# xmarre/person_capture

Hardware: AMD Instinct MI355X
Metric: frames/sec detect+embed+match @1080p, 1/2/4/8 GPU; MFMA util % (higher is better)
Workload: dtype f16x3

## Files before the change

### include/pcgpu.h

```cpp
#ifndef PCGPU_H
#define PCGPU_H

#include <stddef.h>
#include <stdint.h>

#ifdef __cplusplus
extern "C" {
#endif

#define PC_ABI_VERSION 1

#define PC_OK 0
#define PC_ERR_ARG 1
#define PC_ERR_HIP 2
#define PC_ERR_STATE 3
#define PC_ERR_FORMAT 4
#define PC_ERR_CAPACITY 5

#define PC_PREC_F16 0
#define PC_PREC_F32 1
#define PC_PREC_F16X3 2

typedef struct pc_ctx pc_ctx;
typedef struct pc_net pc_net;
// ... 79 lines not shown
int pc_host_free(pc_ctx* ctx, void* h_ptr);
int pc_fence_create(pc_ctx* ctx, void** fence_out);
int pc_fence_record(pc_ctx* ctx, void* fence);
int pc_fence_wait(pc_ctx* ctx, void* fence);
int pc_fence_destroy(pc_ctx* ctx, void* fence);

int pc_net_create(pc_ctx* ctx, const void* h_program, size_t program_bytes, int precision, int max_batch,
                  pc_net** out);
int pc_net_destroy(pc_net* net);
int pc_net_run(pc_net* net, const void* d_input, int batch);
int pc_net_input_dims(pc_net* net, int32_t* h_dims4 );
int pc_net_output(pc_net* net, int index, void** d_ptr, int32_t* h_dims5 );
int pc_net_num_outputs(pc_net* net);
int pc_net_stats(pc_net* net, double* h_flops_per_image, int32_t* h_launches);
int pc_net_chain_info(pc_net* net, int32_t* h_min_batch, int32_t* h_images_per_round);
int pc_net_set_chain_min_batch(pc_net* net, int32_t min_batch);
int pc_net_set_graph(pc_net* net, int enable);
int pc_net_set_graph_max_batch(pc_net* net, int32_t max_batch);
int pc_net_profile(pc_net* net, int enable);
int pc_net_calibrate(pc_net* net, const void* d_in, int N, int headroom_log2, float* h_absmax);
int pc_net_profile_read(pc_net* net, double* h_out5);
int pc_net_profile_ops(pc_net* net, double* h_out, int max_recs);

int pc_letterbox(pc_ctx* ctx, int precision, const pc_letterbox_desc* h_descs, int n, int D, void* d_out);
int pc_warp_affine(pc_ctx* ctx, const pc_warp_desc* h_descs, int n);
int pc_resize_linear(pc_ctx* ctx, const pc_resize_desc* h_descs, int n);
int pc_face_quality(pc_ctx* ctx, const uint8_t* d_chips, int n, int side, double* d_out);
int pc_arcface_prep(pc_ctx* ctx, int precision, const uint8_t* d_chips, int n, int side, int flip, void* d_out);
int pc_rotate_pad(pc_ctx* ctx, const uint8_t* d_src, int H, int W, int row_stride, int deg, int pad, uint8_t* d_dst);
int pc_resize_area_fast(pc_ctx* ctx, const uint8_t* d_src, int row_stride, int isx, int isy, uint8_t* d_dst, int OH,
// ... 41 lines not shown
```

### person_capture_amd/_lib.py

```python
from __future__ import annotations

import ctypes as C
import os
from pathlib import Path

LIB_PATH = Path(os.environ.get("PC_LIB_PATH") or Path(__file__).resolve().parent / "lib" / "libpcgpu.so")

PC_OK = 0
PC_PREC_F16 = 0
PC_PREC_F32 = 1
PC_PREC_F16X3 = 2
PC_PREC_F16C8 = 3


def net_precision(mode: int) -> int:
    return PC_PREC_F16 if mode in (PC_PREC_F16X3, PC_PREC_F16C8) else mode

_lib = None


class LetterboxDesc(C.Structure):
    _fields_ = [("d_src", C.c_void_p), ("H", C.c_int32), ("W", C.c_int32), ("row_stride", C.c_int32),
                ("new_w", C.c_int32), ("new_h", C.c_int32), ("scale_x", C.c_double), ("scale_y", C.c_double),
                ("simd_end", C.c_int32), ("pad_", C.c_int32)]
# ... 61 lines not shown
    "pc_fence_create": ([_P, C.POINTER(_P)], _I),
    "pc_fence_record": ([_P, _P], _I),
    "pc_fence_wait": ([_P, _P], _I),
    "pc_fence_destroy": ([_P, _P], _I),
    "pc_net_create": ([_P, _P, _SZ, _I, _I, C.POINTER(_P)], _I),
    "pc_net_destroy": ([_P], _I),
    "pc_net_run": ([_P, _P, _I], _I),
    "pc_net_input_dims": ([_P, C.POINTER(C.c_int32)], _I),
    "pc_net_output": ([_P, _I, C.POINTER(_P), C.POINTER(C.c_int32)], _I),
    "pc_net_num_outputs": ([_P], _I),
    "pc_net_stats": ([_P, C.POINTER(C.c_double), C.POINTER(C.c_int32)], _I),
    "pc_ctx_wait_fence": ([_P, _P], _I),
    "pc_frame_stage": ([_P, _P, _P, C.c_size_t, C.c_size_t, C.c_size_t, C.c_int], _I),
    "pc_net_chain_info": ([_P, C.POINTER(C.c_int32), C.POINTER(C.c_int32)], _I),
    "pc_net_set_chain_min_batch": ([_P, C.c_int32], _I),
    "pc_net_set_graph": ([_P, _I], _I),
    "pc_net_set_graph_max_batch": ([_P, C.c_int32], _I),
    "pc_net_profile": ([_P, _I], _I),
    "pc_net_calibrate": ([_P, _P, _I, _I, C.POINTER(C.c_float)], _I),
    "pc_net_profile_read": ([_P, C.POINTER(C.c_double)], _I),
    "pc_net_profile_ops": ([_P, C.POINTER(C.c_double), _I], _I),
    "pc_letterbox": ([_P, _I, C.POINTER(LetterboxDesc), _I, _I, _P], _I),
    "pc_warp_affine": ([_P, C.POINTER(WarpDesc), _I], _I),
    "pc_resize_linear": ([_P, C.POINTER(ResizeDesc), _I], _I),
    "pc_face_quality": ([_P, _P, _I, _I, _P], _I),
    "pc_arcface_prep": ([_P, _I, _P, _I, _I, _I, _P], _I),
    "pc_rotate_pad": ([_P, _P, _I, _I, _I, _I, _I, _P], _I),
    "pc_resize_area_fast": ([_P, _P, _I, _I, _I, _P, _I, _I], _I),
    "pc_resize_area": ([_P, _P, _I, C.POINTER(AreaTab), C.POINTER(C.c_int32), _I, C.POINTER(AreaTab),
                        C.POINTER(C.c_int32), _I, _P, _I, _I], _I),
# ... 54 lines not shown
```

### person_capture_amd/csrc/pc_api.cpp

```cpp
#include <hip/hip_runtime.h>
#include <string.h>
#include <stdio.h>
#include <stdlib.h>
#include <string>
#include <vector>
#include <map>
#include <algorithm>
#include <thread>
#include <mutex>
#include <memory>
#include <cmath>
#include <atomic>
#include <condition_variable>
#include <functional>
#include <system_error>
#include "../../include/pcgpu.h"
#include "pc_common.h"

namespace pc {
hipError_t conv_launch(int f32, int rowb, int cfg, const ConvParams& p, hipStream_t s);
hipError_t conv_halo_launch(int f32, int cfg, const ConvParams& p, hipStream_t s);
hipError_t conv_fast_launch(int f32, int rowb, int cfg, const ConvParams& p, hipStream_t s);
hipError_t conv_hx_launch(const ConvParams& p, hipStream_t s);
hipError_t conv_hxg_launch(const ConvParams& p, int small, hipStream_t s);
hipError_t conv_hxi_launch(const ConvParams& p, int small, hipStream_t s);
int conv_fast_num_cfgs();
constexpr int kFastSmallCfg0 = 15, kFastSmallCfg1 = 19;
int conv_fast_tile(int cfg, int* bc, int* bp);
int conv_fast_valid(int cfg, int rowb);
int conv_fast_valid_sx(int cfg, int rowb);
int conv_fast_valid_c8(int cfg, int rowb);
int conv_fast_valid_wg(int cfg);
int conv_halo_num_cfgs();
int conv_halo_tile(int cfg, int* bc, int* bp);
int conv_halo_fits(int cfg, int KH, int KW, int W);
hipError_t conv_t2d_launch(const ConvParams& p, int variant, hipStream_t s);
int conv_t2d_select(int cin, int npad, int KH, int KW, int stride, int pad, int act, int out_f32, int ycs,
                    int ycoff, int split);
int conv_t2d_rows(int variant);
int conv_chain_fits(int H, int W, int C, int npad, long long ktot);
// ... 481 lines not shown
  int split = 0;
  void* w = nullptr;
  float* bias = nullptr;
  float* slope = nullptr;
};
struct ProfRec { int a, b, kind; double flops; int op = -1; int code = -1; int small = -1; };
struct ChainBlockH { const void* w1; const float* b1; const float* s1; const void* w2; const float* b2; };
struct ChainPlan {
  int first = -1, nblk = 0, in_t = -1, out_t = -1;
  void* d_blk = nullptr;
  void* d_wpack = nullptr;
  int wl = 0;
  double flops_per_image = 0.0;
};

struct pc_net {
  pc_ctx* ctx = nullptr;
  int f32 = 0;
  int max_batch = 0;
  int in_tensor = 0;
  int in_centered = 0;
  std::vector<NetBuf> bufs;
  std::vector<NetTensor> tens;
  std::vector<NetOp> ops;
  std::vector<int> outs;
  std::vector<void*> arrays;
  std::vector<long long> array_count;
  std::vector<ConvPlan> plans;
  std::vector<std::vector<ConvPlan>> plans_cls;
  std::vector<int> cls_batch;
  std::vector<StemPlan> stems;
  std::vector<ChainPlan> chains;
  std::vector<int> chain_at;
  int chain_min_batch = 32;
  int attn_stream = 0;
  std::vector<const float*> host_arrays;
  void* stem_col = nullptr;
  float* partial = nullptr;
  size_t partial_bytes = 0;
  double flops_per_image = 0.0;
  int launches = 0;
  const void* cur_input = nullptr;
  void* in_copy = nullptr;
  size_t in_img_bytes = 0;
  int use_graph = 0;
  int capturing = 0;
  hipStream_t cap_stream = nullptr;
  std::mutex graph_mu;
  int graph_max_batch = 1 << 30;
// ... 19 lines not shown
    return (void*)(base + (size_t)T.coff * esize(n, T.is_f32));
  }
  return (char*)n->bufs[T.buf].d + (size_t)T.coff * esize(n, T.is_f32);
}

static const size_t kZeroTail = 65536;

static unsigned tensor_zero_off(const pc_net* n, int t) {
  const NetTensor& T = n->tens[t];
  const int es = esize(n, T.is_f32);
  const size_t end = T.buf < 0 ? n->in_img_bytes * n->max_batch : (size_t)n->bufs[T.buf].elems * n->max_batch * es;
  return (unsigned)(end - (size_t)T.coff * es);
}

static const int kNumConvCfgs = 14;

static int c8_rowb() {
  const char* e = getenv("PC_C8_ROWB");
  return e && atoi(e) == 128 ? 128 : 64;
}

static int plan_conv(pc_net* n, const NetOp& op, ConvPlan& pl, long long plan_batch, bool small = false) {
  const int* w = op.w;
  const int out = w[1], nseg = w[2], npad = w[14];
  const int esz = n->f32 ? 4 : 2;
  int rowb = 128;
  bool any_split = n->tens[out].split != 0 || (w[21] >= 0 && n->tens[w[21]].split);
  for (int s = 0; s < nseg; ++s) {
    const NetTensor& X = n->tens[w[3 + 5 * s]];
    const int cl = X.split ? X.C / 2 : X.C;
// ... 174 lines not shown
    }
    const bool c224 = X.C == 448 && Y.H == 20 && plan_batch <= 16;
    if (X.split && !X.c8 && !Y.c8 && (X.C == 192 || c224) && X.cs == X.C && Y.split && Y.C == X.C && npad == X.C / 2 &&
        w[4] == 3 && w[5] == 3 && w[6] == 1 && w[7] == 1 && X.H == Y.H && X.W == Y.W && w[15] == 27 * npad &&
        !(w[21] >= 0 && (w[22] == RES_UP2 || !n->tens[w[21]].split || n->tens[w[21]].c8)) &&
        (double)X.H * X.W * n->max_batch * X.cs * esz + kZeroTail < 4294967296.0 &&
        !(getenv("PC_CONV_HXG") && atoi(getenv("PC_CONV_HXG")) == 0)) {
      const int hxg_mask = getenv("PC_CONV_HXG") ? atoi(getenv("PC_CONV_HXG")) : 3;
      if (plan_batch * ((Y.H + 19) / 20) * ((Y.W + 15) / 16) >= 128 && (hxg_mask & 1) && !c224) pl.hx = 2;
      else if ((hxg_mask & 2) && (Y.H >= 40 || plan_batch <= 16)) pl.hx = 5;
    }
    if (pl.hx == 2 || pl.hx == 5) {
      pl.fast = pl.halo = pl.t2d = -1;
      pl.sx = 0;
    }
    const int hxi_mask = getenv("PC_CONV_HXI") ? atoi(getenv("PC_CONV_HXI")) : 59;
    if (!X.split && !X.c8 && !X.is_f32 && !Y.split && !Y.is_f32 && !Y.c8 && X.cs == X.C && Y.cs == Y.C && Y.C == X.C &&
        npad == X.C && w[4] == 3 && w[5] == 3 && w[6] == 1 && w[7] == 1 && X.W == X.H && Y.H == X.H && Y.W == X.W &&
        w[15] == 9 * X.C && !(w[21] >= 0 && (w[22] == RES_UP2 || n->tens[w[21]].split || n->tens[w[21]].is_f32)) &&
        (((hxi_mask & 4) && X.C == 256 && X.H == 14 && plan_batch >= 192) ||
         ((hxi_mask & 8) && X.C == 128 && X.H == 28 && plan_batch >= 64)) &&
        (double)X.H * X.W * n->max_batch * X.cs * esz + kZeroTail < 4294967296.0) {
      pl.hx = X.C == 256 ? 3 : 4;
      pl.fast = pl.halo = pl.t2d = -1;
      pl.sx = 0;
    }
    const int hc = X.C / 2;
    const bool hxs_shape = (hxi_mask & 32) && plan_batch <= 32 &&
                           ((hc == 256 && X.H == 14) || (hc == 128 && X.H == 28) || (hc == 512 && X.H == 7));
    const bool hxi_shape = ((hxi_mask & 1) && hc == 256 && X.H == 14 && plan_batch >= 192) ||
                           ((hxi_mask & 2) && hc == 128 && X.H == 28 && plan_batch >= 64) ||
// ... 187 lines not shown
    }
    for (int k = 0; k < ch.nblk; ++k) {
      const int* a = n->ops[i + 2 * k].w;
      const int* b = n->ops[i + 2 * k + 1].w;
      const void* w1 = ch.wl ? (const void*)((char*)ch.d_wpack + cbytes * (2 * k)) : n->arrays[a[13]];
      const void* w2 = ch.wl ? (const void*)((char*)ch.d_wpack + cbytes * (2 * k + 1)) : n->arrays[b[13]];
      hb[k] = ChainBlockH{w1, (const float*)n->arrays[a[17]], (const float*)n->arrays[a[19]], w2,
                          (const float*)n->arrays[b[17]]};
      ch.flops_per_image += n->plans[i + 2 * k].flops_per_image + n->plans[i + 2 * k + 1].flops_per_image;
    }
    HIPCHK(n->ctx, hipMalloc(&ch.d_blk, hb.size() * sizeof(ChainBlockH)));
    HIPCHK(n->ctx, hipMemcpy(ch.d_blk, hb.data(), hb.size() * sizeof(ChainBlockH), hipMemcpyHostToDevice));
    n->chain_at[i] = (int)n->chains.size();
    n->chains.push_back(ch);
    i += 2 * ch.nblk;
  }
  return PC_OK;
}

static uint8_t e4m3_encode(float v) {
  const uint8_t sgn = std::signbit(v) ? 0x80 : 0;
  const float a = std::fabs(v);
  if (!(a == a)) return 0x7f;
  if (a >= 448.f) return sgn | 0x7e;
  int e2 = 0;
  std::frexp(a, &e2);
  int E = e2 - 1;
  if (a == 0.f || E < -6) {
    const int q = (int)std::nearbyint(std::ldexp(a, 9));
    return sgn | (uint8_t)q;
// ... 306 lines not shown
      n->flops_per_image += 4.0 * T * T * op.w[3] * op.w[4];
      n->launches += 1;
    } else {
      rc = fail(c, PC_ERR_FORMAT, "unknown op type");
    }
  }
  n->wfrag.assign(n->ops.size(), nullptr);
  for (size_t i = 0; i < n->ops.size() && rc == PC_OK; ++i) {
    if (n->ops[i].w[0] != OP_CONV) continue;
    bool wg = n->plans[i].wg || n->plans[i].hx;
    for (auto& pc : n->plans_cls) wg = wg || pc[i].wg || pc[i].hx;
    if (wg) rc = pack_wfrag(n, n->ops[i], reinterpret_cast<const float*>(n->host_arrays[n->ops[i].w[13]]), &n->wfrag[i]);
  }
  n->host_arrays.clear();
  if (rc == PC_OK) rc = plan_chains(n);
  if (rc == PC_OK && stem_col_bytes) {
    if (hipMalloc(&n->stem_col, stem_col_bytes) != hipSuccess) rc = fail(c, PC_ERR_HIP, "stem im2col workspace");
    else hipMemset(n->stem_col, 0, stem_col_bytes);
  }
  if (rc == PC_OK && part) {
    if (hipMalloc((void**)&n->partial, part) != hipSuccess) rc = fail(c, PC_ERR_HIP, "split-K workspace");
    n->partial_bytes = part;
  }
  if (rc != PC_OK) {
    pc_net_destroy(n);
    return rc;
  }
  *out = n;
  return PC_OK;
}
// ... 5 lines not shown
  for (auto& kv : n->graphs) hipGraphExecDestroy(kv.second);
  if (n->cap_stream) hipStreamDestroy(n->cap_stream);
  if (n->d_absmax) hipFree(n->d_absmax);
  for (void* a : n->arrays) if (a) hipFree(a);
  for (void* a : n->wfrag) if (a) hipFree(a);
  for (auto& b : n->bufs) if (b.d) hipFree(b.d);
  if (n->partial) hipFree(n->partial);
  if (n->prep) hipFree(n->prep);
  if (n->in_copy) hipFree(n->in_copy);
  for (auto& st : n->stems) {
    if (st.w) hipFree(st.w);
    if (st.bias) hipFree(st.bias);
    if (st.slope) hipFree(st.slope);
  }
  if (n->stem_col) hipFree(n->stem_col);
  for (auto& ch : n->chains) {
    if (ch.d_blk) hipFree(ch.d_blk);
    if (ch.d_wpack) hipFree(ch.d_wpack);
  }
  delete n;
  return PC_OK;
}

static int prof_event(pc_net* n, int* idx) {
  if (n->ev_used == n->ev_pool.size()) {
    hipEvent_t e;
    HIPCHK(n->ctx, hipEventCreate(&e));
    n->ev_pool.push_back(e);
  }
  *idx = (int)n->ev_used++;
  HIPCHK(n->ctx, hipEventRecord(n->ev_pool[*idx], n->ctx->stream));
  return PC_OK;
}

static int plan_class(const pc_net* n, int N) {
  for (size_t c = 0; c < n->cls_batch.size(); ++c)
    if (N <= n->cls_batch[c]) return (int)c;
  return -1;
}

static int run_ops(pc_net* n, int N, hipStream_t s) {
  pc_ctx* c = n->ctx;
  const bool prof = n->prof && !n->capturing;
  if (n->in_copy)
    HIPCHK(c, hipMemcpyAsync(n->in_copy, n->cur_input, n->in_img_bytes * N, hipMemcpyDeviceToDevice, s));
  int open_ev = -1;
  for (size_t i = 0; i < n->ops.size(); ++i) {
    const int* w = n->ops[i].w;
    if (!n->chain_at.empty() && n->chain_at[i] >= 0 && N >= n->chain_min_batch) {
      const ChainPlan& ch = n->chains[n->chain_at[i]];
      ProfRec rec{-1, -1, OP_CONV, ch.flops_per_image * N, (int)i, 300};
      if (prof) {
        if (open_ev >= 0) {
// ... 8 lines not shown
      int mode = 1;
      if (const char* e = getenv("PC_CHAIN_MODE")) mode = atoi(e) ? 1 : 0;
      dbg |= mode << 10;
      if (const char* e = getenv("PC_CONV_DBG")) dbg |= atoi(e) & 7;
      HIPCHK(c, conv_chain_launch(tensor_ptr(n, ch.in_t), TX.cs, tensor_ptr(n, ch.out_t), TY.cs, ch.d_blk, ch.nblk, N,
                                  TX.H, TX.W, n->ops[i].w[15], dbg, s));
      if (prof) {
        int rc = prof_event(n, &rec.b);
        if (rc) return rc;
        n->recs.push_back(rec);
        open_ev = rec.b;
      }
      i += 2 * ch.nblk - 1;
      continue;
    }
    ProfRec rec{-1, -1, w[0], w[0] == OP_CONV ? n->plans[i].flops_per_image * N : 0.0, (int)i};
    if (prof) {
      if (open_ev >= 0) {
        rec.a = open_ev;
      } else {
        int rc = prof_event(n, &rec.a);
        if (rc) return rc;
      }
    }
    if (w[0] == OP_CONV) {
      const int cls = plan_class(n, N);
      const ConvPlan& pl = cls >= 0 ? n->plans_cls[cls][i] : n->plans[i];
      rec.small = cls;
      ConvParams p;
      memset(&p, 0, sizeof(p));
      const NetTensor& Y = n->tens[w[1]];
      p.nseg = w[2];
      const int bke = pl.rowb / (n->f32 ? 4 : 2);
      int kt = 0;
      for (int sg = 0; sg < p.nseg; ++sg) {
        const NetTensor& X = n->tens[w[3 + 5 * sg]];
        ConvSeg& S = p.seg[sg];
        S.x = tensor_ptr(n, w[3 + 5 * sg]);
        S.zero_off = tensor_zero_off(n, w[3 + 5 * sg]);
        S.H = X.H; S.W = X.W; S.C = X.C; S.cs = X.cs;
        S.KH = w[4 + 5 * sg]; S.KW = w[5 + 5 * sg]; S.stride = w[6 + 5 * sg]; S.pad = w[7 + 5 * sg];
        S.cblk = X.C / bke;
        if (X.c8) S.f8s = (127 - X.e_lo) | ((127 - X.e_hi) << 8);
        if (X.split && pl.sx) {
          S.cblk = S.cblk / 2;
          S.vwrap = S.cblk;
          S.gt = (X.C / 2) % 64 == 0 ? 64 / bke : 1;
        } else if (X.split) {
          S.vwrap = S.cblk;
          S.cblk = S.cblk / 2 * 3;
        }
        S.kt = S.KH * S.KW * S.cblk;
        kt += S.kt;
      }
      p.w = n->arrays[w[13]];
      p.ktot = w[15];
      p.N = N; p.OH = Y.H; p.OW = Y.W; p.M = N * Y.H * Y.W;
      p.npad = w[14];
      p.cout = w[16];
      p.cwrite = std::min(Y.split ? Y.C / 2 : Y.C, p.npad);
      p.ysplit = Y.split ? Y.C / 2 : 0;
      p.y = tensor_ptr(n, w[1]);
      p.ycs = Y.cs;
      p.out_f32 = Y.is_f32 && !n->f32 ? 1 : (n->f32 ? 1 : 0);
      p.bias = w[17] >= 0 ? (const float*)n->arrays[w[17]] : nullptr;
      p.bias_mode = w[17] >= 0 ? w[18] : 0;
      p.slope = w[19] >= 0 ? (const float*)n->arrays[w[19]] : nullptr;
      p.act = w[20];
      p.res = w[21] >= 0 ? tensor_ptr(n, w[21]) : nullptr;
      p.res_mode = w[21] >= 0 ? w[22] : 0;
      if (w[21] >= 0) {
        const NetTensor& R = n->tens[w[21]];
        p.rcs = R.cs; p.rH = R.H; p.rW = R.W;
        p.rsplit = R.split ? R.C / 2 : 0;
      }
      p.act_after_res = w[23];
      p.kt_total = kt;
      p.sx = pl.sx;
      p.c8 = pl.c8;
      p.wf8s = n->wf8s[i];
      p.wfrag = pl.wg || pl.hx ? n->wfrag[i] : nullptr;
      if (Y.c8) {
        p.yc8 = 1;
        p.ylo_mul = std::ldexp(1.f, Y.e_lo);
        p.yhi_mul = std::ldexp(1.f, Y.e_hi);
      }
      if (w[21] >= 0 && n->tens[w[21]].c8) {
        p.rc8 = 1;
        p.rlo_inv = std::ldexp(1.f, -n->tens[w[21]].e_lo);
      }
      p.splitk = pl.splitk;
      p.partial = n->partial;
      p.zero = c->zero;
      if (const char* e = getenv("PC_CONV_DBG")) p.dbg = atoi(e);
      if (pl.hx >= 3 && pl.hx != 5) {
        HIPCHK(c, conv_hxi_launch(p, pl.hx >= 7, s));
      } else if (pl.hx == 2 || pl.hx == 5) {
        HIPCHK(c, conv_hxg_launch(p, pl.hx == 5, s));
      } else if (pl.hx) {
        HIPCHK(c, conv_hx_launch(p, s));
      } else if (pl.t2d >= 0) {
        HIPCHK(c, conv_t2d_launch(p, pl.t2d, s));
      } else if (pl.fast >= 0) {
        HIPCHK(c, conv_fast_launch(n->f32, pl.rowb, pl.fast, p, s));
      } else if (pl.halo >= 0) {
        HIPCHK(c, conv_halo_launch(n->f32, pl.halo, p, s));
      } else {
        HIPCHK(c, conv_launch(n->f32, pl.rowb, pl.cfg, p, s));
      }
      if (pl.splitk > 1) {
        HIPCHK(c, splitk_finish_launch(n->f32, p, s));
// ... 106 lines not shown
      p.qlo = Q.split ? Q.C / 2 : 0;
      p.olo = O.split ? O.C / 2 : 0;
      HIPCHK(c, attention_launch(n->f32, p, w[4], n->attn_stream, s));
    }
    if (n->calib && (w[0] == OP_CONV || w[0] == OP_STEM)) {
      const NetTensor& Y = n->tens[w[1]];
      if (!Y.is_f32 && !n->f32)
        HIPCHK(c, absmax_f16_launch(tensor_ptr(n, w[1]), (long long)N * Y.H * Y.W, Y.split ? Y.C / 2 : Y.C, Y.cs,
                                    reinterpret_cast<unsigned*>(n->d_absmax) + w[1], s));
    }
    if (prof) {
      int rc = prof_event(n, &rec.b);
      if (rc) return rc;
      n->recs.push_back(rec);
      open_ev = rec.b;
    }
  }
  return PC_OK;
}

extern "C" int pc_net_calibrate(pc_net* n, const void* d_in, int N, int headroom_log2, float* h_absmax) {
  if (!n || !d_in || N <= 0 || N > n->max_batch || headroom_log2 < 0 || headroom_log2 > 8) return PC_ERR_ARG;
  pc_ctx* c = n->ctx;
  std::lock_guard<std::mutex> lk(n->graph_mu);
  const size_t nt = n->tens.size();
  if (!n->d_absmax) HIPCHK(c, hipMalloc((void**)&n->d_absmax, nt * 4));
  HIPCHK(c, hipMemsetAsync(n->d_absmax, 0, nt * 4, c->stream));
  n->cur_input = d_in;
  n->calib = 1;
  const int rc = run_ops(n, N, c->stream);
// ... 640 lines not shown
```

### person_capture_amd/csrc/pc_conv_hxi.hip

```cpp
#include "pc_conv_common.h"

#include <cstdlib>

namespace pc {

template <int HW, int PITCH, int ROWS, int CIN, int COUT, int WCH, int WPX, bool SPLIT, int OCC>
struct HxiGeom {
  static constexpr int NW = WCH * WPX, NT = 64 * NW;
  static constexpr int NF = (ROWS * PITCH + 15) / 16;
  static constexpr int TP = NF / WPX, TC = COUT / WCH / 16;
  static constexpr int CB = CIN / COUT;
  static constexpr int WPS = (NW * OCC + 3) / 4;
  static constexpr int TPG = WPS > 2 ? 1 : (TP > 7 ? (TP % 2 == 0 ? TP / 2 : TP) : TP);
  static constexpr int WD = WPS == 1 ? 6 : 2;
  static constexpr bool PF = WPS == 1 && SPLIT && TPG == TP;
  static constexpr int SB = SPLIT ? 256 : CIN * 2;
  static constexpr int NB = SPLIT ? 2 : CIN / 32;
  static constexpr int NG = SPLIT ? CIN / 64 : 1, KPG = 9 * NB, NKS = NG * KPG;
  static constexpr int SLOTS = (NF * 16 > ROWS * PITCH ? NF * 16 - ROWS * PITCH : 0) + (ROWS + 2) * PITCH + 2;
  static constexpr int PIECES = (SLOTS * SB + 1023) / 1024;
  static constexpr int STAGE = PIECES * 1024;
  static constexpr int NSTAGE = NG > 1 && 2 * STAGE * OCC <= 163840 ? 2 : 1;
  static constexpr int NPIX = ROWS * HW;
  static constexpr int PC = COUT * NPIX * 4 <= 131072 / OCC ? COUT : COUT / 2;
  static constexpr int NPASS = COUT / PC;
  static constexpr int RS = PC + 4;
  static constexpr int EPI = NPIX * RS * 4;
  static constexpr int SMEM = NSTAGE * STAGE > EPI ? NSTAGE * STAGE : EPI;
  static constexpr int WTILE = SPLIT ? 2048 : 1024;
  static constexpr int CGN = PC / 8;
  static constexpr int IT = (NPIX + NT / CGN - 1) / (NT / CGN);
  static_assert(PITCH >= HW + 2 && NF % WPX == 0 && TP % TPG == 0, "pixel fragments");
  static_assert(COUT % (16 * WCH) == 0 && CIN % 64 == 0 && HW % ROWS == 0 && SB % 256 == 0, "tiling");
  static_assert(SMEM <= 163840, "LDS");
  static_assert(NPASS == 1 || WCH % 2 == 0, "epilogue passes split the channel waves");
};

template <int HW, int PITCH, int ROWS, int CIN, int COUT, int WCH, int WPX, bool SPLIT = true, int OCC = 1>
__global__ __launch_bounds__(64 * WCH * WPX, (WCH * WPX * OCC + 3) / 4) void conv_hxi(ConvParams p) {
  using G = HxiGeom<HW, PITCH, ROWS, CIN, COUT, WCH, WPX, SPLIT, OCC>;
  constexpr int NW = G::NW, NT = G::NT, TC = G::TC, TP = G::TP, TPG = G::TPG, NG = G::NG, NKS = G::NKS;
  constexpr int STAGE = G::STAGE, PIECES = G::PIECES, SB = G::SB, NB = G::NB, KPG = G::KPG;
  static_assert(G::SMEM * OCC <= 163840, "LDS for OCC workgroups per CU");
  static_assert(NW <= 16, "waves");
  __shared__ __attribute__((aligned(16))) char smem[G::SMEM];
  const ConvSeg& S = p.seg[0];
  const int lane = threadIdx.x & 63;
  const int wave = __builtin_amdgcn_readfirstlane(threadIdx.x >> 6);
  const int wch = wave % WCH, wpx = wave / WCH;
  constexpr int RB = HW / ROWS, CB = G::CB;
  const int b = xcd_remap(blockIdx.x, p.N * RB * CB);
  const int cb = b % CB, nb = b / CB;
  const int n = nb / RB, r0 = (nb - n * RB) * ROWS;
  const int fr = lane & 15, kg = lane >> 4;

  auto rsrc = [](const void* base) __attribute__((always_inline)) {
    return __builtin_amdgcn_make_buffer_rsrc(const_cast<void*>(base), (short)0, (int)0xffffffff, 0x00020000);
  };
  const __amdgpu_buffer_rsrc_t xrs = rsrc(S.x);
  const __amdgpu_buffer_rsrc_t wrs = rsrc(p.wfrag);

  constexpr int PPW = (PIECES + NW - 1) / NW;
  auto stage = [&](int g, int st) __attribute__((always_inline)) {
#pragma unroll
    for (int j = 0; j < PPW; ++j) {
      if (wave + NW * j < PIECES) {
// ... 141 lines not shown
      });
    });
  });
  asm volatile("s_waitcnt vmcnt(0)" ::: "memory");
  if (p.dbg & 4) return;

  constexpr int NPIX = G::NPIX, RS = G::RS, PC = G::PC, NPASS = G::NPASS, CGN = G::CGN, IT = G::IT;
  static_assert(NT % CGN == 0, "a thread keeps one 8-channel group");
  constexpr int PSTEP = NT / CGN;
  float* im = reinterpret_cast<float*>(smem);
  const bool smooth = p.act == ACT_SILU || p.act == ACT_GELU;
  const bool has_res = p.res_mode != RES_NONE;
  const bool pre_act = !p.act_after_res;
  const bool border = p.bias_mode == BIAS_BORDER9;
  const long long pix0 = (long long)n * HW * HW + r0 * HW;
  const int cg = threadIdx.x % CGN, pl0 = threadIdx.x / CGN;
#pragma unroll
  for (int pass = 0; pass < NPASS; ++pass) {
    const int ch = cb * COUT + pass * PC + cg * 8;
    float bc[8], sl[8];
#pragma unroll
    for (int j = 0; j < 8; ++j) {
      bc[j] = p.bias_mode == BIAS_CHANNEL ? p.bias[ch + j] : 0.f;
      sl[j] = p.act == ACT_PRELU ? p.slope[ch + j] : (p.act == ACT_RELU ? 0.f : 1.f);
    }
    constexpr bool PREF = G::WPS <= 2;
    float pre[PREF ? IT : 1][8];
    auto load_pre = [&](int k, float* dst) __attribute__((always_inline)) {
      const int pl = pl0 + PSTEP * k;
#pragma unroll
      for (int j = 0; j < 8; ++j) dst[j] = 0.f;
// ... 86 lines not shown
      f16x8 yh, yl;
#pragma unroll
      for (int j = 0; j < 8; ++j) {
        const float x = ch + j < p.cout ? v[j] : 0.f;
        yh[j] = (f16)x;
        yl[j] = (f16)(x - (float)yh[j]);
      }
      if (p.dbg & 16) continue;
      f16* yp = reinterpret_cast<f16*>(p.y) + pix * p.ycs + ch;
      *reinterpret_cast<f16x8*>(yp) = yh;
      if constexpr (SPLIT) *reinterpret_cast<f16x8*>(yp + p.ysplit) = yl;
    }
  }
}

#define PC_HXI_14 14, 16, 14, 256, 256, 8, 1
#define PC_HXI_28 28, 32, 7, 128, 128, 4, 2
#define PC_HXI_7 7, 9, 7, 512, 512, 8, 1
#define PC_HXI_14S 14, 16, 7, 256, 32, 2, 1
#define PC_HXI_28S 28, 32, 7, 128, 32, 2, 2
#define PC_HXI_7S 7, 9, 7, 512, 32, 2, 1

int conv_hxi_ok(const ConvParams& p) {
  const ConvSeg& S = p.seg[0];
  const bool split = p.ysplit != 0;
  const int C = split ? S.C / 2 : S.C, w = split ? 2 : 1;
  const bool shape = (S.H == 14 && C == 256) || (S.H == 28 && C == 128) || (split && S.H == 7 && C == 512);
  return shape && p.nseg == 1 && S.cs == w * C && S.W == S.H && S.KH == 3 && S.KW == 3 && S.stride == 1 &&
         S.pad == 1 && p.OH == S.H && p.OW == S.H && p.npad == C && p.ycs == w * C && p.splitk == 1 && !p.out_f32 &&
         !p.yc8 && !p.rc8 && p.ktot == 9 * (split ? 3 : 1) * C && p.res_mode != RES_UP2 &&
         (p.res_mode == RES_NONE || (p.rsplit == (split ? C : 0) && p.rcs % 8 == 0)) && p.cwrite == C &&
         p.wfrag != nullptr && (!split || p.ysplit == C);
}

hipError_t conv_hxi_launch(const ConvParams& p, int small, hipStream_t s) {
  if (!conv_hxi_ok(p)) return hipErrorInvalidValue;
  const bool split = p.ysplit != 0;
  if (small) {
    if (!split) return hipErrorInvalidValue;
    const dim3 grid(p.N * 16);
    if (p.OH == 7) hipLaunchKernelGGL((conv_hxi<PC_HXI_7S, true, 2>), grid, dim3(128), 0, s, p);
    else if (p.OH == 14) hipLaunchKernelGGL((conv_hxi<PC_HXI_14S, true, 2>), grid, dim3(128), 0, s, p);
    else hipLaunchKernelGGL((conv_hxi<PC_HXI_28S, true, 1>), grid, dim3(256), 0, s, p);
  } else if (p.OH == 7) {
    hipLaunchKernelGGL((conv_hxi<PC_HXI_7, true, 1>), dim3(p.N), dim3(512), 0, s, p);
  } else if (p.OH == 14) {
    if (split) hipLaunchKernelGGL((conv_hxi<PC_HXI_14, true, 1>), dim3(p.N), dim3(512), 0, s, p);
    else hipLaunchKernelGGL((conv_hxi<PC_HXI_14, false, 1>), dim3(p.N), dim3(512), 0, s, p);
  } else {
    const bool occ1 = getenv("PC_HXI28_OCC") && atoi(getenv("PC_HXI28_OCC")) == 1;
    if (split && occ1) hipLaunchKernelGGL((conv_hxi<PC_HXI_28, true, 1>), dim3(p.N * 4), dim3(512), 0, s, p);
    else if (split) hipLaunchKernelGGL((conv_hxi<PC_HXI_28, true, 2>), dim3(p.N * 4), dim3(512), 0, s, p);
    else hipLaunchKernelGGL((conv_hxi<PC_HXI_28, false, 2>), dim3(p.N * 4), dim3(512), 0, s, p);
  }
  return hipGetLastError();
}

}
```

Measured before the change: 1014.

## Fuse consecutive per-image hxi 3x3 convs into one persistent chain kernel

Adds a planner that finds runs of consecutive eligible split-f16 3x3 convs at 14x14 or 7x7, where each layer feeds the next and intermediate tensors are not used outside the run. Each run is executed by one kernel that loops over the layers with one workgroup per image, reading the per-layer params from device constant memory and separating layers with a workgroup barrier. This removes per-layer launch overhead and lets a layer's output stay in cache for the next layer. It also turns the per-launch getenv for the 28x28 occupancy choice into a value read once at setup. In exchange the chain kernel runs at occupancy 1 with the grid fixed to the batch size, and profiling records for fused layers become placeholders.

```diff
diff --git a/include/pcgpu.h b/include/pcgpu.h
--- a/include/pcgpu.h
+++ b/include/pcgpu.h
@@ -117,6 +117,8 @@
 int pc_net_num_outputs(pc_net* net);
 int pc_net_stats(pc_net* net, double* h_flops_per_image, int32_t* h_launches);
 int pc_net_chain_info(pc_net* net, int32_t* h_min_batch, int32_t* h_images_per_round);
+int pc_plan_hxi_runs(const int32_t* h_ops, int n_ops, const int32_t* h_eligible, const int32_t* h_outs, int n_outs,
+                     int cap, int32_t* h_runs, int max_runs);
 int pc_net_set_chain_min_batch(pc_net* net, int32_t min_batch);
 int pc_net_set_graph(pc_net* net, int enable);
 int pc_net_set_graph_max_batch(pc_net* net, int32_t max_batch);
diff --git a/person_capture_amd/_lib.py b/person_capture_amd/_lib.py
--- a/person_capture_amd/_lib.py
+++ b/person_capture_amd/_lib.py
@@ -99,6 +99,8 @@
     "pc_frame_stage": ([_P, _P, _P, C.c_size_t, C.c_size_t, C.c_size_t, C.c_int], _I),
     "pc_net_chain_info": ([_P, C.POINTER(C.c_int32), C.POINTER(C.c_int32)], _I),
     "pc_net_set_chain_min_batch": ([_P, C.c_int32], _I),
+    "pc_plan_hxi_runs": ([C.POINTER(C.c_int32), _I, C.POINTER(C.c_int32), C.POINTER(C.c_int32), _I, _I,
+                          C.POINTER(C.c_int32), _I], _I),
     "pc_net_set_graph": ([_P, _I], _I),
     "pc_net_set_graph_max_batch": ([_P, C.c_int32], _I),
     "pc_net_profile": ([_P, _I], _I),
diff --git a/person_capture_amd/csrc/pc_api.cpp b/person_capture_amd/csrc/pc_api.cpp
--- a/person_capture_amd/csrc/pc_api.cpp
+++ b/person_capture_amd/csrc/pc_api.cpp
@@ -23,7 +23,9 @@
 hipError_t conv_fast_launch(int f32, int rowb, int cfg, const ConvParams& p, hipStream_t s);
 hipError_t conv_hx_launch(const ConvParams& p, hipStream_t s);
 hipError_t conv_hxg_launch(const ConvParams& p, int small, hipStream_t s);
-hipError_t conv_hxi_launch(const ConvParams& p, int small, hipStream_t s);
+hipError_t conv_hxi_launch(const ConvParams& p, int small, int occ1_28, hipStream_t s);
+int conv_hxi_chain_ok(const ConvParams& p);
+hipError_t conv_hxi_chain_launch(const void* d_layers, int nl, int HW, int N, hipStream_t s);
 int conv_fast_num_cfgs();
 constexpr int kFastSmallCfg0 = 15, kFastSmallCfg1 = 19;
 int conv_fast_tile(int cfg, int* bc, int* bp);
@@ -535,6 +537,17 @@
   double flops_per_image = 0.0;
 };
 
+struct HxiRun {
+  int first = -1, nl = 0, hw = 0;
+  size_t param_off = 0;
+  double flops_per_image = 0.0;
+};
+struct HxiRuns {
+  std::vector<HxiRun> runs;
+  std::vector<int> at;
+  void* d_params = nullptr;
+};
+
 struct pc_net {
   pc_ctx* ctx = nullptr;
   int f32 = 0;
@@ -554,6 +567,9 @@
   std::vector<ChainPlan> chains;
   std::vector<int> chain_at;
   int chain_min_batch = 32;
+  std::vector<HxiRuns> hxi_runs;
+  int hxi_chain_max = 8;
+  int hxi28_occ1 = 0;
   int attn_stream = 0;
   std::vector<const float*> host_arrays;
   void* stem_col = nullptr;
@@ -603,6 +619,7 @@
 }
 
 static const int kNumConvCfgs = 14;
+static const int kHxiDefaultMask = 123;
 
 static int c8_rowb() {
   const char* e = getenv("PC_C8_ROWB");
@@ -807,7 +824,7 @@
       pl.fast = pl.halo = pl.t2d = -1;
       pl.sx = 0;
     }
-    const int hxi_mask = getenv("PC_CONV_HXI") ? atoi(getenv("PC_CONV_HXI")) : 59;
+    const int hxi_mask = getenv("PC_CONV_HXI") ? atoi(getenv("PC_CONV_HXI")) : kHxiDefaultMask;
     if (!X.split && !X.c8 && !X.is_f32 && !Y.split && !Y.is_f32 && !Y.c8 && X.cs == X.C && Y.cs == Y.C && Y.C == X.C &&
         npad == X.C && w[4] == 3 && w[5] == 3 && w[6] == 1 && w[7] == 1 && X.W == X.H && Y.H == X.H && Y.W == X.W &&
         w[15] == 9 * X.C && !(w[21] >= 0 && (w[22] == RES_UP2 || n->tens[w[21]].split || n->tens[w[21]].is_f32)) &&
@@ -1025,6 +1042,122 @@
     n->chain_at[i] = (int)n->chains.size();
     n->chains.push_back(ch);
     i += 2 * ch.nblk;
+  }
+  return PC_OK;
+}
+
+static void find_hxi_runs(const int32_t* ops, int nops, const int32_t* elig, const int32_t* outs, int nouts,
+                          int cap, std::vector<std::pair<int, int>>& launches) {
+  launches.clear();
+  auto W = [&](int i) { return ops + (size_t)i * 32; };
+  int nt = 0;
+  auto reads = [&](int i, auto&& fn) {
+    const int32_t* w = W(i);
+    if (w[0] == OP_CONV) {
+      for (int sg = 0; sg < w[2] && sg < 2; ++sg) fn(w[3 + 5 * sg]);
+      if (w[21] >= 0) fn(w[21]);
+    } else {
+      fn(w[2]);
+    }
+  };
+  for (int i = 0; i < nops; ++i) {
+    nt = std::max(nt, W(i)[1] + 1);
+    reads(i, [&](int t) { nt = std::max(nt, t + 1); });
+  }
+  for (int k = 0; k < nouts; ++k) nt = std::max(nt, outs[k] + 1);
+  const int kNever = -1, kAlways = 1 << 30;
+  std::vector<int> last_use(nt, kNever), producer(nt, kNever);
+  for (int i = 0; i < nops; ++i) {
+    reads(i, [&](int t) { if (t >= 0) last_use[t] = std::max(last_use[t], i); });
+    if (W(i)[1] >= 0) producer[W(i)[1]] = i;
+  }
+  for (int k = 0; k < nouts; ++k) if (outs[k] >= 0) last_use[outs[k]] = kAlways;
+  auto res_ok = [&](int i) { const int r = W(i)[21]; return r < 0 || producer[r] < i; };
+  auto follows = [&](int i) {
+    const int32_t* w = W(i);
+    return elig[i] && w[0] == OP_CONV && w[2] == 1 && w[3] == W(i - 1)[1] && res_ok(i);
+  };
+  for (int f = 0; f < nops;) {
+    if (!elig[f] || W(f)[0] != OP_CONV || W(f)[2] != 1 || !res_ok(f)) { ++f; continue; }
+    int e = f;
+    while (e + 1 < nops && follows(e + 1)) ++e;
+    int j = e;
+    for (; j > f; --j) {
+      bool ok = true;
+      for (int i = f; i < j && ok; ++i) ok = last_use[W(i)[1]] <= j;
+      if (ok) break;
+    }
+    const int L = j - f + 1, step = cap > 0 ? cap : L;
+    for (int o = 0; o < L; o += step) launches.emplace_back(f + o, std::min(step, L - o));
+    f = j + 1;
+  }
+}
+
+extern "C" int pc_plan_hxi_runs(const int32_t* ops, int n_ops, const int32_t* eligible, const int32_t* outs,
+                                int n_outs, int cap, int32_t* runs, int max_runs) {
+  if (!ops || !eligible || n_ops < 0 || (n_outs > 0 && !outs) || (max_runs > 0 && !runs)) return -PC_ERR_ARG;
+  std::vector<std::pair<int, int>> l;
+  find_hxi_runs(ops, n_ops, eligible, outs, n_outs, cap, l);
+  for (size_t k = 0; k < l.size() && (int)k < max_runs; ++k) {
+    runs[2 * k] = l[k].first;
+    runs[2 * k + 1] = l[k].second;
+  }
+  return (int)l.size();
+}
+
+static void conv_params(pc_net* n, size_t i, const ConvPlan& pl, int N, ConvParams& p);
+
+static int plan_hxi_runs(pc_net* n) {
+  n->hxi_runs.clear();
+  if (const char* e = getenv("PC_HXI28_OCC")) n->hxi28_occ1 = atoi(e) == 1;
+  if (const char* e = getenv("PC_HXI_CHAIN_MAX")) n->hxi_chain_max = std::max(0, atoi(e));
+  const int hxi_mask = getenv("PC_CONV_HXI") ? atoi(getenv("PC_CONV_HXI")) : kHxiDefaultMask;
+  if (n->f32 || !(hxi_mask & 64) || getenv("PC_CONV_DBG")) return PC_OK;
+  const int nops = (int)n->ops.size();
+  std::vector<int32_t> words((size_t)nops * 32), elig(nops);
+  for (int i = 0; i < nops; ++i) memcpy(&words[(size_t)i * 32], n->ops[i].w, sizeof(n->ops[i].w));
+  std::vector<int32_t> outs(n->outs.begin(), n->outs.end());
+  n->hxi_runs.resize(1 + n->plans_cls.size());
+  for (size_t k = 0; k < n->hxi_runs.size(); ++k) {
+    const std::vector<ConvPlan>& plans = k ? n->plans_cls[k - 1] : n->plans;
+    HxiRuns& R = n->hxi_runs[k];
+    R.at.assign(nops, -1);
+    std::vector<ConvParams> params(nops);
+    bool any = false;
+    for (int i = 0; i < nops; ++i) {
+      elig[i] = 0;
+      const int* w = n->ops[i].w;
+      if (w[0] != OP_CONV || (plans[i].hx != 3 && plans[i].hx != 6) || plans[i].splitk != 1) continue;
+      const NetTensor &X = n->tens[w[3]], &Y = n->tens[w[1]];
+      bool ok = X.buf >= 0 && Y.buf >= 0 && X.split && Y.split && X.H == Y.H && X.W == Y.W && X.cs == Y.cs;
+      if (ok && w[21] >= 0) {
+        const NetTensor& T = n->tens[w[21]];
+        ok = T.buf >= 0 && T.H == Y.H && T.W == Y.W && T.cs == Y.cs;
+      }
+      if (!ok) continue;
+      conv_params(n, i, plans[i], 0, params[i]);
+      elig[i] = conv_hxi_chain_ok(params[i]);
+      any = any || elig[i];
+    }
+    if (!any) continue;
+    std::vector<std::pair<int, int>> launches;
+    find_hxi_runs(words.data(), nops, elig.data(), outs.data(), (int)outs.size(), n->hxi_chain_max, launches);
+    std::vector<ConvParams> packed;
+    for (auto& l : launches) {
+      HxiRun r;
+      r.first = l.first;
+      r.nl = l.second;
+      r.hw = n->tens[n->ops[l.first].w[1]].H;
+      r.param_off = packed.size();
+      for (int i = l.first; i < l.first + l.second; ++i) {
+        packed.push_back(params[i]);
+        r.flops_per_image += n->plans[i].flops_per_image;
+      }
+      R.at[l.first] = (int)R.runs.size();
+      R.runs.push_back(r);
+    }
+    HIPCHK(n->ctx, hipMalloc(&R.d_params, packed.size() * sizeof(ConvParams)));
+    HIPCHK(n->ctx, hipMemcpy(R.d_params, packed.data(), packed.size() * sizeof(ConvParams), hipMemcpyHostToDevice));
   }
   return PC_OK;
 }
@@ -1361,6 +1494,7 @@
   }
   n->host_arrays.clear();
   if (rc == PC_OK) rc = plan_chains(n);
+  if (rc == PC_OK) rc = plan_hxi_runs(n);
   if (rc == PC_OK && stem_col_bytes) {
     if (hipMalloc(&n->stem_col, stem_col_bytes) != hipSuccess) rc = fail(c, PC_ERR_HIP, "stem im2col workspace");
     else hipMemset(n->stem_col, 0, stem_col_bytes);
@@ -1396,6 +1530,7 @@
     if (st.slope) hipFree(st.slope);
   }
   if (n->stem_col) hipFree(n->stem_col);
+  for (auto& R : n->hxi_runs) if (R.d_params) hipFree(R.d_params);
   for (auto& ch : n->chains) {
     if (ch.d_blk) hipFree(ch.d_blk);
     if (ch.d_wpack) hipFree(ch.d_wpack);
@@ -1419,6 +1554,75 @@
   for (size_t c = 0; c < n->cls_batch.size(); ++c)
     if (N <= n->cls_batch[c]) return (int)c;
   return -1;
+}
+
+static void conv_params(pc_net* n, size_t i, const ConvPlan& pl, int N, ConvParams& p) {
+  pc_ctx* c = n->ctx;
+  const int* w = n->ops[i].w;
+  memset(&p, 0, sizeof(p));
+  const NetTensor& Y = n->tens[w[1]];
+  p.nseg = w[2];
+  const int bke = pl.rowb / (n->f32 ? 4 : 2);
+  int kt = 0;
+  for (int sg = 0; sg < p.nseg; ++sg) {
+    const NetTensor& X = n->tens[w[3 + 5 * sg]];
+    ConvSeg& S = p.seg[sg];
+    S.x = tensor_ptr(n, w[3 + 5 * sg]);
+    S.zero_off = tensor_zero_off(n, w[3 + 5 * sg]);
+    S.H = X.H; S.W = X.W; S.C = X.C; S.cs = X.cs;
+    S.KH = w[4 + 5 * sg]; S.KW = w[5 + 5 * sg]; S.stride = w[6 + 5 * sg]; S.pad = w[7 + 5 * sg];
+    S.cblk = X.C / bke;
+    if (X.c8) S.f8s = (127 - X.e_lo) | ((127 - X.e_hi) << 8);
+    if (X.split && pl.sx) {
+      S.cblk = S.cblk / 2;
+      S.vwrap = S.cblk;
+      S.gt = (X.C / 2) % 64 == 0 ? 64 / bke : 1;
+    } else if (X.split) {
+      S.vwrap = S.cblk;
+      S.cblk = S.cblk / 2 * 3;
+    }
+    S.kt = S.KH * S.KW * S.cblk;
+    kt += S.kt;
+  }
+  p.w = n->arrays[w[13]];
+  p.ktot = w[15];
+  p.N = N; p.OH = Y.H; p.OW = Y.W; p.M = N * Y.H * Y.W;
+  p.npad = w[14];
+  p.cout = w[16];
+  p.cwrite = std::min(Y.split ? Y.C / 2 : Y.C, p.npad);
+  p.ysplit = Y.split ? Y.C / 2 : 0;
+  p.y = tensor_ptr(n, w[1]);
+  p.ycs = Y.cs;
+  p.out_f32 = Y.is_f32 && !n->f32 ? 1 : (n->f32 ? 1 : 0);
+  p.bias = w[17] >= 0 ? (const float*)n->arrays[w[17]] : nullptr;
+  p.bias_mode = w[17] >= 0 ? w[18] : 0;
+  p.slope = w[19] >= 0 ? (const float*)n->arrays[w[19]] : nullptr;
+  p.act = w[20];
+  p.res = w[21] >= 0 ? tensor_ptr(n, w[21]) : nullptr;
+  p.res_mode = w[21] >= 0 ? w[22] : 0;
+  if (w[21] >= 0) {
+    const NetTensor& R = n->tens[w[21]];
+    p.rcs = R.cs; p.rH = R.H; p.rW = R.W;
+    p.rsplit = R.split ? R.C / 2 : 0;
+  }
+  p.act_after_res = w[23];
+  p.kt_total = kt;
+  p.sx = pl.sx;
+  p.c8 = pl.c8;
+  p.wf8s = n->wf8s[i];
+  p.wfrag = pl.wg || pl.hx ? n->wfrag[i] : nullptr;
+  if (Y.c8) {
+    p.yc8 = 1;
+    p.ylo_mul = std::ldexp(1.f, Y.e_lo);
+    p.yhi_mul = std::ldexp(1.f, Y.e_hi);
+  }
+  if (w[21] >= 0 && n->tens[w[21]].c8) {
+    p.rc8 = 1;
+    p.rlo_inv = std::ldexp(1.f, -n->tens[w[21]].e_lo);
+  }
+  p.splitk = pl.splitk;
+  p.partial = n->partial;
+  p.zero = c->zero;
 }
 
 static int run_ops(pc_net* n, int N, hipStream_t s) {
@@ -1457,7 +1661,11 @@
       i += 2 * ch.nblk - 1;
       continue;
     }
-    ProfRec rec{-1, -1, w[0], w[0] == OP_CONV ? n->plans[i].flops_per_image * N : 0.0, (int)i};
+    const int cls = plan_class(n, N);
+    const HxiRuns* hr = n->hxi_runs.empty() ? nullptr : &n->hxi_runs[cls + 1];
+    const HxiRun* run = hr && !n->calib && !hr->runs.empty() && hr->at[i] >= 0 ? &hr->runs[hr->at[i]] : nullptr;
+    ProfRec rec{-1, -1, w[0], run ? run->flops_per_image * N : w[0] == OP_CONV ? n->plans[i].flops_per_image * N : 0.0,
+                (int)i, run ? 300 : -1};
     if (prof) {
       if (open_ev >= 0) {
         rec.a = open_ev;
@@ -1466,78 +1674,18 @@
         if (rc) return rc;
       }
     }
-    if (w[0] == OP_CONV) {
-      const int cls = plan_class(n, N);
+    if (run) {
+      rec.small = cls;
+      HIPCHK(c, conv_hxi_chain_launch(static_cast<const ConvParams*>(hr->d_params) + run->param_off, run->nl, run->hw, N, s));
+      i += run->nl - 1;
+    } else if (w[0] == OP_CONV) {
       const ConvPlan& pl = cls >= 0 ? n->plans_cls[cls][i] : n->plans[i];
       rec.small = cls;
       ConvParams p;
-      memset(&p, 0, sizeof(p));
-      const NetTensor& Y = n->tens[w[1]];
-      p.nseg = w[2];
-      const int bke = pl.rowb / (n->f32 ? 4 : 2);
-      int kt = 0;
-      for (int sg = 0; sg < p.nseg; ++sg) {
-        const NetTensor& X = n->tens[w[3 + 5 * sg]];
-        ConvSeg& S = p.seg[sg];
-        S.x = tensor_ptr(n, w[3 + 5 * sg]);
-        S.zero_off = tensor_zero_off(n, w[3 + 5 * sg]);
-        S.H = X.H; S.W = X.W; S.C = X.C; S.cs = X.cs;
-        S.KH = w[4 + 5 * sg]; S.KW = w[5 + 5 * sg]; S.stride = w[6 + 5 * sg]; S.pad = w[7 + 5 * sg];
-        S.cblk = X.C / bke;
-        if (X.c8) S.f8s = (127 - X.e_lo) | ((127 - X.e_hi) << 8);
-        if (X.split && pl.sx) {
-          S.cblk = S.cblk / 2;
-          S.vwrap = S.cblk;
-          S.gt = (X.C / 2) % 64 == 0 ? 64 / bke : 1;
-        } else if (X.split) {
-          S.vwrap = S.cblk;
-          S.cblk = S.cblk / 2 * 3;
-        }
-        S.kt = S.KH * S.KW * S.cblk;
-        kt += S.kt;
-      }
-      p.w = n->arrays[w[13]];
-      p.ktot = w[15];
-      p.N = N; p.OH = Y.H; p.OW = Y.W; p.M = N * Y.H * Y.W;
-      p.npad = w[14];
-      p.cout = w[16];
-      p.cwrite = std::min(Y.split ? Y.C / 2 : Y.C, p.npad);
-      p.ysplit = Y.split ? Y.C / 2 : 0;
-      p.y = tensor_ptr(n, w[1]);
-      p.ycs = Y.cs;
-      p.out_f32 = Y.is_f32 && !n->f32 ? 1 : (n->f32 ? 1 : 0);
-      p.bias = w[17] >= 0 ? (const float*)n->arrays[w[17]] : nullptr;
-      p.bias_mode = w[17] >= 0 ? w[18] : 0;
-      p.slope = w[19] >= 0 ? (const float*)n->arrays[w[19]] : nullptr;
-      p.act = w[20];
-      p.res = w[21] >= 0 ? tensor_ptr(n, w[21]) : nullptr;
-      p.res_mode = w[21] >= 0 ? w[22] : 0;
-      if (w[21] >= 0) {
-        const NetTensor& R = n->tens[w[21]];
-        p.rcs = R.cs; p.rH = R.H; p.rW = R.W;
-        p.rsplit = R.split ? R.C / 2 : 0;
-      }
-      p.act_after_res = w[23];
-      p.kt_total = kt;
-      p.sx = pl.sx;
-      p.c8 = pl.c8;
-      p.wf8s = n->wf8s[i];
-      p.wfrag = pl.wg || pl.hx ? n->wfrag[i] : nullptr;
-      if (Y.c8) {
-        p.yc8 = 1;
-        p.ylo_mul = std::ldexp(1.f, Y.e_lo);
-        p.yhi_mul = std::ldexp(1.f, Y.e_hi);
-      }
-      if (w[21] >= 0 && n->tens[w[21]].c8) {
-        p.rc8 = 1;
-        p.rlo_inv = std::ldexp(1.f, -n->tens[w[21]].e_lo);
-      }
-      p.splitk = pl.splitk;
-      p.partial = n->partial;
-      p.zero = c->zero;
+      conv_params(n, i, pl, N, p);
       if (const char* e = getenv("PC_CONV_DBG")) p.dbg = atoi(e);
       if (pl.hx >= 3 && pl.hx != 5) {
-        HIPCHK(c, conv_hxi_launch(p, pl.hx >= 7, s));
+        HIPCHK(c, conv_hxi_launch(p, pl.hx >= 7, n->hxi28_occ1, s));
       } else if (pl.hx == 2 || pl.hx == 5) {
         HIPCHK(c, conv_hxg_launch(p, pl.hx == 5, s));
       } else if (pl.hx) {
@@ -1674,6 +1822,8 @@
       if (rc) return rc;
       n->recs.push_back(rec);
       open_ev = rec.b;
+      for (int k = 1; run && k < run->nl; ++k)
+        n->recs.push_back(ProfRec{rec.b, rec.b, OP_CONV, 0.0, rec.op + k, 301, cls});
     }
   }
   return PC_OK;
diff --git a/person_capture_amd/csrc/pc_conv_hxi.hip b/person_capture_amd/csrc/pc_conv_hxi.hip
--- a/person_capture_amd/csrc/pc_conv_hxi.hip
+++ b/person_capture_amd/csrc/pc_conv_hxi.hip
@@ -1,6 +1,4 @@
 #include "pc_conv_common.h"
-
-#include <cstdlib>
 
 namespace pc {
 
@@ -36,20 +34,19 @@
   static_assert(NPASS == 1 || WCH % 2 == 0, "epilogue passes split the channel waves");
 };
 
-template <int HW, int PITCH, int ROWS, int CIN, int COUT, int WCH, int WPX, bool SPLIT = true, int OCC = 1>
-__global__ __launch_bounds__(64 * WCH * WPX, (WCH * WPX * OCC + 3) / 4) void conv_hxi(ConvParams p) {
+template <int HW, int PITCH, int ROWS, int CIN, int COUT, int WCH, int WPX, bool SPLIT, int OCC, class P>
+__device__ __forceinline__ void conv_hxi_layer(P& p, const int N, const int tid, char* smem) {
   using G = HxiGeom<HW, PITCH, ROWS, CIN, COUT, WCH, WPX, SPLIT, OCC>;
   constexpr int NW = G::NW, NT = G::NT, TC = G::TC, TP = G::TP, TPG = G::TPG, NG = G::NG, NKS = G::NKS;
   constexpr int STAGE = G::STAGE, PIECES = G::PIECES, SB = G::SB, NB = G::NB, KPG = G::KPG;
   static_assert(G::SMEM * OCC <= 163840, "LDS for OCC workgroups per CU");
   static_assert(NW <= 16, "waves");
-  __shared__ __attribute__((aligned(16))) char smem[G::SMEM];
-  const ConvSeg& S = p.seg[0];
-  const int lane = threadIdx.x & 63;
-  const int wave = __builtin_amdgcn_readfirstlane(threadIdx.x >> 6);
+  auto& S = p.seg[0];
+  const int lane = tid & 63;
+  const int wave = __builtin_amdgcn_readfirstlane(tid >> 6);
   const int wch = wave % WCH, wpx = wave / WCH;
   constexpr int RB = HW / ROWS, CB = G::CB;
-  const int b = xcd_remap(blockIdx.x, p.N * RB * CB);
+  const int b = xcd_remap(blockIdx.x, N * RB * CB);
   const int cb = b % CB, nb = b / CB;
   const int n = nb / RB, r0 = (nb - n * RB) * ROWS;
   const int fr = lane & 15, kg = lane >> 4;
@@ -221,7 +218,7 @@
   const bool pre_act = !p.act_after_res;
   const bool border = p.bias_mode == BIAS_BORDER9;
   const long long pix0 = (long long)n * HW * HW + r0 * HW;
-  const int cg = threadIdx.x % CGN, pl0 = threadIdx.x / CGN;
+  const int cg = tid % CGN, pl0 = tid / CGN;
 #pragma unroll
   for (int pass = 0; pass < NPASS; ++pass) {
     const int ch = cb * COUT + pass * PC + cg * 8;
@@ -338,6 +335,30 @@
   }
 }
 
+template <int HW, int PITCH, int ROWS, int CIN, int COUT, int WCH, int WPX, bool SPLIT = true, int OCC = 1>
+__global__ __launch_bounds__(64 * WCH * WPX, (WCH * WPX * OCC + 3) / 4) void conv_hxi(ConvParams p) {
+  __shared__ __attribute__((aligned(16))) char smem[HxiGeom<HW, PITCH, ROWS, CIN, COUT, WCH, WPX, SPLIT, OCC>::SMEM];
+  conv_hxi_layer<HW, PITCH, ROWS, CIN, COUT, WCH, WPX, SPLIT, OCC>(p, p.N, (int)threadIdx.x, smem);
+}
+
+template <int HW, int PITCH, int ROWS, int CIN, int COUT, int WCH, int WPX>
+__global__ __launch_bounds__(64 * WCH * WPX, (WCH * WPX + 3) / 4) void conv_hxi_chain(const ConvParams* lp, int nl) {
+  __shared__ __attribute__((aligned(16))) char smem[HxiGeom<HW, PITCH, ROWS, CIN, COUT, WCH, WPX, true, 1>::SMEM];
+  typedef const __attribute__((address_space(4))) ConvParams CP;
+  CP* cp = (CP*)lp;
+  for (int l = 0; l < nl; ++l) {
+    if (l) {
+      asm volatile("s_waitcnt vmcnt(0)" ::: "memory");
+      __builtin_amdgcn_fence(__ATOMIC_RELEASE, "workgroup");
+      __syncthreads();
+      __builtin_amdgcn_fence(__ATOMIC_ACQUIRE, "workgroup");
+    }
+    int tid = threadIdx.x;
+    asm volatile("" : "+v"(tid));
+    conv_hxi_layer<HW, PITCH, ROWS, CIN, COUT, WCH, WPX, true, 1>(cp[l], (int)gridDim.x, tid, smem);
+  }
+}
+
 #define PC_HXI_14 14, 16, 14, 256, 256, 8, 1
 #define PC_HXI_28 28, 32, 7, 128, 128, 4, 2
 #define PC_HXI_7 7, 9, 7, 512, 512, 8, 1
@@ -357,7 +378,7 @@
          p.wfrag != nullptr && (!split || p.ysplit == C);
 }
 
-hipError_t conv_hxi_launch(const ConvParams& p, int small, hipStream_t s) {
+hipError_t conv_hxi_launch(const ConvParams& p, int small, int occ1_28, hipStream_t s) {
   if (!conv_hxi_ok(p)) return hipErrorInvalidValue;
   const bool split = p.ysplit != 0;
   if (small) {
@@ -372,12 +393,24 @@
     if (split) hipLaunchKernelGGL((conv_hxi<PC_HXI_14, true, 1>), dim3(p.N), dim3(512), 0, s, p);
     else hipLaunchKernelGGL((conv_hxi<PC_HXI_14, false, 1>), dim3(p.N), dim3(512), 0, s, p);
   } else {
-    const bool occ1 = getenv("PC_HXI28_OCC") && atoi(getenv("PC_HXI28_OCC")) == 1;
-    if (split && occ1) hipLaunchKernelGGL((conv_hxi<PC_HXI_28, true, 1>), dim3(p.N * 4), dim3(512), 0, s, p);
+    if (split && occ1_28) hipLaunchKernelGGL((conv_hxi<PC_HXI_28, true, 1>), dim3(p.N * 4), dim3(512), 0, s, p);
     else if (split) hipLaunchKernelGGL((conv_hxi<PC_HXI_28, true, 2>), dim3(p.N * 4), dim3(512), 0, s, p);
     else hipLaunchKernelGGL((conv_hxi<PC_HXI_28, false, 2>), dim3(p.N * 4), dim3(512), 0, s, p);
   }
   return hipGetLastError();
 }
 
-}
+int conv_hxi_chain_ok(const ConvParams& p) {
+  return conv_hxi_ok(p) && p.ysplit != 0 && (p.OH == 14 || p.OH == 7) && p.dbg == 0;
+}
+
+hipError_t conv_hxi_chain_launch(const void* d_layers, int nl, int HW, int N, hipStream_t s) {
+  if (!d_layers || nl < 1 || N < 1) return hipErrorInvalidValue;
+  const ConvParams* lp = static_cast<const ConvParams*>(d_layers);
+  if (HW == 14) hipLaunchKernelGGL((conv_hxi_chain<PC_HXI_14>), dim3(N), dim3(512), 0, s, lp, nl);
+  else if (HW == 7) hipLaunchKernelGGL((conv_hxi_chain<PC_HXI_7>), dim3(N), dim3(512), 0, s, lp, nl);
+  else return hipErrorInvalidValue;
+  return hipGetLastError();
+}
+
+}
```

Result: faster. 1041 (median of 6 runs) (+2.7%).
